# NeuralRevenant/RASSEngine

Measured on AMD Instinct MI355X. Metric: queries/sec, exact cosine top-10 over N x 1024-d fp32 corpus in HBM, higher is better.
Workload: dtype f32; 1 GPU; 1000000 x 1024-d flat cosine top-10, 1 x MI355X, precomputed embeddings (BASELINE configs[1]); rows_per_gpu=1000000, rows_global=1000000, dim=1024, k=10, query_batch=32, corpus_dtype=f32, layout=tile16, mode=flat

## Files before the change

include/rass_engine.h:

```cpp
#ifndef RASS_ENGINE_H
#define RASS_ENGINE_H

#include <stddef.h>
#include <stdint.h>

#ifdef __cplusplus
extern "C" {
#endif

#define RASS_ABI_VERSION 1

typedef enum rass_status {
    RASS_OK = 0,
    RASS_ERR_INVALID = -1,
    RASS_ERR_HIP = -2,
    RASS_ERR_OOM = -3,
    RASS_ERR_NOT_FOUND = -4,
    RASS_ERR_UNSUPPORTED = -5,
    RASS_ERR_IO = -6
} rass_status;

typedef enum rass_dtype {
    RASS_F32 = 0,
    RASS_BF16 = 1,
// ... 178 lines not shown
                                     const int32_t* d_q_filter, const int32_t* d_q_filter_mask,
                                     int64_t id_base, int32_t* d_out_groups, int64_t* d_out_counts, float* d_out_scores,
                                     int64_t* d_out_ids, int64_t* d_n_buckets, int64_t* d_total_hits, int32_t* d_status);

int rass_index_rows_gram(rass_index_t* idx, const int64_t* rows, int n_lists, int list_len, float* out);
int rass_index_rows_gram_device(rass_index_t* idx, const int64_t* d_rows, int n_lists, int list_len, float* d_out);

int rass_index_search_mmr(rass_index_t* idx, const float* queries, int nq, int k, int fetch_k,
                          const float* lambda, const int32_t* q_filter, const int32_t* q_filter_mask,
                          float* out_scores, int64_t* out_ids, int32_t* out_rank);
int rass_index_search_mmr_device(rass_index_t* idx, const float* d_queries, int nq, int k, int fetch_k,
                                 const float* d_lambda, const int32_t* d_q_filter, const int32_t* d_q_filter_mask,
                                 int64_t id_base, float* d_out_scores, int64_t* d_out_ids, int32_t* d_out_rank);

#define RASS_PREFILTER_OFF 0
#define RASS_PREFILTER_BF16 1
#define RASS_PREFILTER_INT8 2
#define RASS_PREFILTER_INT8_EXACT 3
int rass_index_set_prefilter(rass_index_t* idx, int enable);
int rass_index_get_prefilter(const rass_index_t* idx);
int rass_index_certify_stats(rass_index_t* idx, int64_t* queries, int64_t* certified, int64_t* fallbacks, float* R, float* V);
int rass_index_candidates_exact_device(rass_index_t* idx, const float* d_queries, int nq, int k, const int32_t* d_q_filter,
                                       float* d_cand_scores, int64_t* d_cand_rows, float* d_tau, int32_t* d_certified);
int rass_index_candidates_device(rass_index_t* idx, const float* d_queries, int nq, const int32_t* d_q_filter,
                                 float* d_cand_scores, int64_t* d_cand_rows);

int rass_index_save(rass_index_t* idx, const char* path);
int rass_index_load(rass_engine_t* eng, const char* name, const char* path,
                    rass_index_t** out);

int rass_index_fill_synthetic(rass_index_t* idx, int64_t n, uint64_t seed,
                              int64_t row_id_base);


size_t rass_scan_workspace_bytes(int nq, int k);

int rass_pack_rows_f32(const float* d_in, int64_t in_stride, float* d_packed,
                       int64_t row_stride, int64_t first_row, int64_t n, int dim,
                       int normalize, void* stream);
int rass_unpack_rows_f32(const float* d_packed, int64_t row_stride,
                         int64_t first_row, int64_t n, int dim, float* d_out,
                         int64_t out_stride, void* stream);
int rass_gather_rows_f32(const float* d_packed, int64_t row_stride, int64_t n_rows,
                         const int64_t* d_row_ids, int64_t n, int dim, float* d_out,
                         int64_t out_stride, void* stream);
int rass_compact_plan(const int32_t* d_tags, int64_t n_rows, int64_t* d_new_row,
// ... 191 lines not shown
```

rassengine_amd/_native.py:

```python
from __future__ import annotations

import ctypes
import os
from typing import Optional

_HERE = os.path.dirname(os.path.abspath(__file__))
LIB_PATH = os.environ.get("RASS_HIP_LIB") or os.path.join(_HERE, "lib", "librass_hip.so")

RASS_OK = 0
RASS_MAX_K = 32
RASS_MAX_K_MULTIPASS = 4096
RASS_TAG_PATIENT_MASK = 0x00FFFFFF
RASS_TAG_DOCTYPE_SHIFT = 24
RASS_TAG_DOCTYPE_MASK = 0x7F000000
RASS_MAX_QBATCH = 32
RASS_MAX_DEVICE_BATCH = 4096
RASS_MAX_MMR_FETCH = 128
RASS_F32 = 0
RASS_BF16 = 1
RASS_QFILTER_NONE = -1
RASS_MAX_ATTRS = 8
RASS_ATTR_MISSING = -(1 << 31)
RASS_MAX_ATTR_CLAUSES = 64
RASS_ATTR_ALL, RASS_ATTR_ANY = 0, 1
# ... 100 lines not shown
    "rass_index_attr_minmax": (ctypes.c_int, [ctypes.c_void_p, ctypes.c_int, ctypes.c_void_p, ctypes.c_void_p, ctypes.c_void_p]),
    "rass_index_search_grouped_keys": (ctypes.c_int, [ctypes.c_void_p, ctypes.c_void_p, ctypes.c_int, ctypes.c_int, ctypes.c_void_p, ctypes.c_int64, ctypes.c_int32, ctypes.c_void_p, ctypes.c_int, ctypes.c_int64, ctypes.c_void_p, ctypes.c_void_p, ctypes.c_void_p, ctypes.c_void_p, ctypes.c_void_p, ctypes.c_void_p]),
    "rass_index_search_grouped_keys_device": (ctypes.c_int, [ctypes.c_void_p, ctypes.c_void_p, ctypes.c_int, ctypes.c_int, ctypes.c_void_p, ctypes.c_int64, ctypes.c_int32, ctypes.c_void_p, ctypes.c_int, ctypes.c_int64, ctypes.c_void_p, ctypes.c_void_p, ctypes.c_int64, ctypes.c_void_p, ctypes.c_void_p, ctypes.c_void_p, ctypes.c_void_p, ctypes.c_void_p]),
    "rass_index_aggregate_keys": (ctypes.c_int, [ctypes.c_void_p, ctypes.c_void_p, ctypes.c_int, ctypes.c_void_p, ctypes.c_int, ctypes.c_void_p, ctypes.c_int64, ctypes.c_int32, ctypes.c_void_p, ctypes.c_int, ctypes.c_int64, ctypes.c_void_p, ctypes.c_void_p, ctypes.c_void_p, ctypes.c_void_p, ctypes.c_void_p, ctypes.c_void_p, ctypes.c_void_p, ctypes.c_void_p]),
    "rass_index_aggregate_keys_device": (ctypes.c_int, [ctypes.c_void_p, ctypes.c_void_p, ctypes.c_int, ctypes.c_void_p, ctypes.c_int, ctypes.c_void_p, ctypes.c_int64, ctypes.c_int32, ctypes.c_void_p, ctypes.c_int, ctypes.c_int64, ctypes.c_void_p, ctypes.c_void_p, ctypes.c_int64, ctypes.c_void_p, ctypes.c_void_p, ctypes.c_void_p, ctypes.c_void_p, ctypes.c_void_p, ctypes.c_void_p, ctypes.c_void_p]),
    "rass_index_rows_gram": (ctypes.c_int, [ctypes.c_void_p, ctypes.c_void_p, ctypes.c_int, ctypes.c_int, ctypes.c_void_p]),
    "rass_index_rows_gram_device": (ctypes.c_int, [ctypes.c_void_p, ctypes.c_void_p, ctypes.c_int, ctypes.c_int,
                                                   ctypes.c_void_p]),
    "rass_index_search_mmr": (ctypes.c_int, [ctypes.c_void_p, ctypes.c_void_p, ctypes.c_int, ctypes.c_int, ctypes.c_int,
                                             ctypes.c_void_p, ctypes.c_void_p, ctypes.c_void_p, ctypes.c_void_p, ctypes.c_void_p,
                                             ctypes.c_void_p]),
    "rass_index_search_mmr_device": (ctypes.c_int, [ctypes.c_void_p, ctypes.c_void_p, ctypes.c_int, ctypes.c_int, ctypes.c_int,
                                                    ctypes.c_void_p, ctypes.c_void_p, ctypes.c_void_p, ctypes.c_int64,
                                                    ctypes.c_void_p, ctypes.c_void_p, ctypes.c_void_p]),
    "rass_index_set_prefilter": (ctypes.c_int, [ctypes.c_void_p, ctypes.c_int]),
    "rass_index_get_prefilter": (ctypes.c_int, [ctypes.c_void_p]),
    "rass_index_candidates_device": (ctypes.c_int, [ctypes.c_void_p, ctypes.c_void_p, ctypes.c_int, ctypes.c_void_p,
                                                    ctypes.c_void_p, ctypes.c_void_p]),
    "rass_index_certify_stats": (ctypes.c_int, [ctypes.c_void_p, ctypes.c_void_p, ctypes.c_void_p, ctypes.c_void_p,
                                                ctypes.c_void_p, ctypes.c_void_p]),
    "rass_index_candidates_exact_device": (ctypes.c_int, [ctypes.c_void_p, ctypes.c_void_p, ctypes.c_int, ctypes.c_int,
                                                          ctypes.c_void_p, ctypes.c_void_p, ctypes.c_void_p, ctypes.c_void_p,
                                                          ctypes.c_void_p]),
    "rass_index_save": (ctypes.c_int, [ctypes.c_void_p, ctypes.c_char_p]),
    "rass_index_load": (ctypes.c_int, [ctypes.c_void_p, ctypes.c_char_p, ctypes.c_char_p, c_void_pp]),
    "rass_index_fill_synthetic": (ctypes.c_int, [ctypes.c_void_p, ctypes.c_int64, ctypes.c_uint64,
                                                 ctypes.c_int64]),
    "rass_scan_workspace_bytes": (ctypes.c_size_t, [ctypes.c_int, ctypes.c_int]),
    "rass_scan_topk_f32": (ctypes.c_int, [ctypes.c_void_p, ctypes.c_int64, ctypes.c_int, ctypes.c_int64,
                                          ctypes.c_void_p, ctypes.c_void_p, ctypes.c_int, ctypes.c_void_p,
                                          ctypes.c_int, ctypes.c_int64, ctypes.c_void_p, ctypes.c_void_p,
                                          ctypes.c_void_p, ctypes.c_size_t, ctypes.c_void_p]),
    "rass_pack_rows_f32": (ctypes.c_int, [ctypes.c_void_p, ctypes.c_int64, ctypes.c_void_p, ctypes.c_int64,
                                          ctypes.c_int64, ctypes.c_int64, ctypes.c_int, ctypes.c_int,
                                          ctypes.c_void_p]),
    "rass_unpack_rows_f32": (ctypes.c_int, [ctypes.c_void_p, ctypes.c_int64, ctypes.c_int64, ctypes.c_int64,
                                            ctypes.c_int, ctypes.c_void_p, ctypes.c_int64, ctypes.c_void_p]),
    "rass_gather_rows_f32": (ctypes.c_int, [ctypes.c_void_p, ctypes.c_int64, ctypes.c_int64, ctypes.c_void_p, ctypes.c_int64,
                                            ctypes.c_int, ctypes.c_void_p, ctypes.c_int64, ctypes.c_void_p]),
    "rass_compact_plan": (ctypes.c_int, [ctypes.c_void_p, ctypes.c_int64, ctypes.c_void_p, ctypes.c_void_p, ctypes.c_void_p,
                                         ctypes.c_void_p, ctypes.c_size_t, ctypes.c_void_p]),
    "rass_compact_plan_workspace_bytes": (ctypes.c_size_t, [ctypes.c_int64]),
    "rass_compact_rows_f32": (ctypes.c_int, [ctypes.c_void_p, ctypes.c_void_p, ctypes.c_int64, ctypes.c_void_p, ctypes.c_int64,
                                             ctypes.c_int64, ctypes.c_void_p]),
    "rass_topk_merge": (ctypes.c_int, [ctypes.c_void_p, ctypes.c_void_p, ctypes.c_int, ctypes.c_int, ctypes.c_int,
                                       ctypes.c_void_p, ctypes.c_void_p, ctypes.c_void_p]),
# ... 159 lines not shown
```

rassengine_amd/csrc/api_internal.h:

```cpp
#pragma once

#include <hip/hip_runtime.h>
#include <stdint.h>
#include <stdio.h>
#include <stdlib.h>
#include <string.h>
#include <unistd.h>

#include <algorithm>
#include <atomic>
#include <condition_variable>
#include <map>
#include <mutex>
#include <new>
#include <string>
#include <type_traits>
#include <vector>

#include "../../include/rass_engine.h"
#include "kernels.h"

namespace rass {
namespace host {

// ... 73 lines not shown
    }
};

struct ScratchView {
    float* q_padded;
    float* part_scores;
    int64_t* part_ids;
    unsigned short* q_bf16;
    float* cand_scores;
    int64_t* cand_ids;
    float* sample_best;
    size_t total;
};
ScratchView scratch_layout(unsigned char* base, int nq, int k);

struct BatchView {
    float* q_padded;
    float* part_scores;
    int64_t* part_ids;
    float* sample_best;
    unsigned char* q_small;
    float* cand_scores;
    int64_t* cand_rows;
    size_t total;
    size_t part_per_group;
    float* group_sample(int g) const { return sample_best + (int64_t)g * 32 * rass::kMaxSampleGroups; }
};
BatchView batch_layout(unsigned char* base, int groups, int grid, int k, int64_t stride, bool candidates = false);

struct CertView {
    float* q_padded;
    signed char* q8;
    rass::CertQInfo* qinfo;
    float* sample;
    float* list_s;
    int32_t* list_r;
    int32_t* list_n;
    float* list_floor;
    int64_t* cand_rows;
    float* rr_s;
    int64_t* rr_i;
    float* tau;
    int32_t *fail_idx, *fail_flag, *fail_n;
    float* fb_q;
    int32_t *fb_filter, *fb_mask;
    float* fb_s;
// ... 181 lines not shown
    uint32_t* d_list_mask = nullptr;
    bool any_tags = false;
    int64_t src_rows = 0;
    int64_t src_epoch = -1;
    std::vector<int32_t> pos_of;
    float* d_pair_scores = nullptr;
    int64_t* d_pair_ids = nullptr;
    unsigned char* d_batch = nullptr;
    size_t batch_bytes = 0;
};

namespace rass {
namespace host {

int set_device(const rass_engine* eng);
int index_reserve(rass_index* idx, int64_t need_rows);
void index_free_slabs(rass_index* idx);
int index_attr_ensure(rass_index* idx, int col);
int index_refresh_copies(rass_index* idx, int64_t first, int64_t n, hipStream_t st);

int scan_xcd_skew(int nq, int grid, int n_cus);
int64_t scan_sample_floor_min_share();
bool i8_sample_floor(int64_t rows, int grid);
bool scan_batch_one_sample();
bool scan_batch_pair();
bool ivf_batch_one_launch();

int scan_grid(int64_t tiles, int lists_kept_per_wg, int n_cus);

template <class F>
int timed_launch(rass_engine* eng, hipStream_t st, F&& launch, int extra_groups = 0) {
    const bool timed = eng && eng->ev_on && (size_t)(2 * eng->ev_used + 1) < eng->ev_pool.size();
    if (timed) HIP_TRY(hipEventRecord(eng->ev_pool[2 * eng->ev_used], st));
    const int rc = launch();
    if (rc != RASS_OK) return rc;
    if (timed) {
        HIP_TRY(hipEventRecord(eng->ev_pool[2 * eng->ev_used + 1], st));
        eng->ev_used += 1;
        eng->ev_extra += extra_groups;
    }
    return RASS_OK;
}

inline void as_sample(rass::ScanArgs& s) { s.xcd_skew = 0, s.sample_pass = true; }
inline void as_sample(rass::ScanBf16Args& s) { s.k = 1; }
inline void as_sample(rass::ScanI8Args& s) { s.k = 1; }
template <class Args>
// ... 142 lines not shown
```

rassengine_amd/csrc/api_scan.hip:

```cpp

#include "api_internal.h"

namespace rass {
namespace host {


int scan_xcd_skew(int nq, int grid, int n_cus) {
    struct Skew {
        int b16 = 4, b32 = 0;
        Skew() {
            if (const char* e = getenv("RASS_SCAN_XCD_SKEW")) {
                int a = 0, b = 0;
                const int n = sscanf(e, "%d,%d", &a, &b);
                if (n == 1) b = a;
                if (n >= 1 && a >= 0 && b >= 0 && a <= 4096 && b <= 4096) b16 = a, b32 = b;
            }
        }
    };
    if (grid != n_cus || grid % 8 != 0) return 0;
    static const Skew skew;
    return nq <= 16 ? skew.b16 : skew.b32;
}

int64_t scan_sample_floor_min_share() {
    const char* e = getenv("RASS_SCAN_SAMPLE_FLOOR");
    if (e && e[0] == '0') return 0;
    if (e && e[0] == 'f') return 2;
    return 32;
}

bool i8_sample_floor(int64_t rows, int grid) {
    const char* e = getenv("RASS_I8_SAMPLE_FLOOR");
    const bool force = e && e[0] == 'f';
    if (e && !force && atoi(e) == 0) return false;
    return grid <= rass::kMaxSampleGroups && rows >= (int64_t)(force ? 2 : 8) * 64 * grid;
}

bool scan_batch_one_sample() {
    const char* e = getenv("RASS_SCAN_BATCH_SAMPLE");
    return !(e && e[0] == 'g');
}

bool scan_batch_pair() {
    static const bool on = [] {
        const char* e = getenv("RASS_SCAN_BATCH_PAIR");
        return !(e && e[0] == '0');
    }();
    return on;
}

bool ivf_batch_one_launch() {
    const char* e = getenv("RASS_IVF_BATCH_FINE");
    return !(e && e[0] == 'g');
}


int scan_grid(int64_t tiles, int lists_kept_per_wg, int n_cus) {
    int grid = (int)std::min<int64_t>(std::max<int64_t>(tiles, 1), std::min(n_cus, kMaxGrid));
    if ((int64_t)grid * lists_kept_per_wg > rass::kMergeMaxCandidates) grid = rass::kMergeMaxCandidates / lists_kept_per_wg;
    return grid;
}

ScratchView scratch_layout(unsigned char* base, int nq, int k) {
// ... 1 lines not shown
    ScratchView L;
    L.q_padded = c.take<float>((size_t)RASS_MAX_QBATCH * kMaxStride * sizeof(float));
    L.part_scores = c.take<float>((size_t)kMaxGrid * nq * k * sizeof(float));
    L.part_ids = c.take<int64_t>((size_t)kMaxGrid * nq * k * sizeof(int64_t));
    L.q_bf16 = c.take<unsigned short>((size_t)RASS_MAX_QBATCH * kMaxStride * 2);
    L.cand_scores = c.take<float>((size_t)RASS_MAX_QBATCH * RASS_MAX_K * sizeof(float));
    L.cand_ids = c.take<int64_t>((size_t)RASS_MAX_QBATCH * RASS_MAX_K * sizeof(int64_t));
    L.sample_best = c.take<float>((size_t)rass::kMaxSampleGroups * 32 * sizeof(float));
    L.total = c.off;
    return L;
}

BatchView batch_layout(unsigned char* base, int groups, int grid, int k, int64_t stride, bool candidates) {
    Carver c{base};
    BatchView L;
    L.part_per_group = (size_t)grid * 32 * k;
    L.q_padded = c.take<float>((size_t)groups * 32 * stride * sizeof(float));
    L.part_scores = c.take<float>((size_t)groups * L.part_per_group * sizeof(float));
    L.part_ids = c.take<int64_t>((size_t)groups * L.part_per_group * sizeof(int64_t));
    L.sample_best = c.take<float>((size_t)groups * 32 * rass::kMaxSampleGroups * sizeof(float));
    L.q_small = candidates ? c.take<unsigned char>((size_t)groups * 32 * kMaxStride * 2) : nullptr;
    L.cand_scores = candidates ? c.take<float>((size_t)groups * 32 * k * sizeof(float)) : nullptr;
    L.cand_rows = candidates ? c.take<int64_t>((size_t)groups * 32 * k * sizeof(int64_t)) : nullptr;
    L.total = c.off;
    return L;
}

CertView cert_layout(unsigned char* base, int grid, int64_t stride, int64_t stride_i8, int dim) {
    Carver c{base};
    CertView L;
    const size_t Q = rass::kCertQ, slots = (size_t)grid * Q * rass::kCertWgCap;
    L.q_padded = c.take<float>(4 * Q * stride * sizeof(float));
    L.q8 = c.take<signed char>(2 * Q * stride_i8);
    L.qinfo = c.take<rass::CertQInfo>(Q * sizeof(rass::CertQInfo));
    L.sample = c.take<float>((size_t)rass::kMaxSampleGroups * Q * sizeof(float));
    L.list_s = c.take<float>(slots * sizeof(float));
    L.list_r = c.take<int32_t>(slots * sizeof(int32_t));
    L.list_n = c.take<int32_t>((size_t)grid * Q * sizeof(int32_t));
    L.list_floor = c.take<float>((size_t)grid * Q * sizeof(float));
    L.cand_rows = c.take<int64_t>(Q * rass::kCertC * sizeof(int64_t));
    L.rr_s = c.take<float>(Q * rass::kCertC * sizeof(float));
    L.rr_i = c.take<int64_t>(Q * rass::kCertC * sizeof(int64_t));
    L.tau = c.take<float>(Q * sizeof(float));
    L.fail_idx = c.take<int32_t>(Q * sizeof(int32_t));
    L.fail_flag = c.take<int32_t>(Q * sizeof(int32_t));
    L.fail_n = c.take<int32_t>(sizeof(int32_t));
// ... 394 lines not shown
```

rassengine_amd/csrc/api_search.hip:

```cpp

#include "api_internal.h"

namespace rass {
namespace host {

HostSlot* slot_acquire(rass_engine* eng) {
    std::unique_lock<std::mutex> lk(eng->slot_mu);
    for (;;) {
        for (HostSlot& sl : eng->slots)
            if (!sl.busy) {
                sl.busy = true;
                return &sl;
            }
        eng->slot_cv.wait(lk);
    }
}

void slot_release(rass_engine* eng, HostSlot* sl) {
    {
        std::lock_guard<std::mutex> lk(eng->slot_mu);
        sl->busy = false;
    }
    eng->slot_cv.notify_one();
}
// ... 38 lines not shown
    const IndexView iv = index_view(idx, r.q_filter != nullptr, r.id_base, r.after_score != nullptr);
    r.use(iv);
    if (idx->dtype == RASS_BF16) return bf16_scan_launch(idx, r);
    if (!exact && idx->prefilter == 3 && iv.rows > 0 && !r.after_score && one_pass) return cert_launch(idx, r);
    if (!exact && idx->prefilter && idx->prefilter != 3 && iv.rows > 0 && r.k <= kPrefilterMaxK && !r.after_score)
        return prefilter_launch(idx, r);
    ScanRequest s = scan_request(eng);
    s.corpus = iv.corpus, s.n_rows = iv.rows, s.stride = idx->stride, s.row_tag = iv.row_tag;
    s.queries = r.queries, s.q_dim = idx->dim, s.q_stride = idx->dim, s.nq = r.nq, s.q_filter = r.q_filter;
    s.k = r.k, s.id_base = iv.id_base, s.id_map = iv.id_map, s.out_scores = r.out_scores, s.out_ids = r.out_ids;
    s.timing = eng;
    s.ext.d_q_mask = r.q_filter_mask, s.ext.d_after_s = r.after_score, s.ext.d_after_i = r.after_row;
    return scan_launch(s);
}

FlatRequest batch_group(const rass_index* idx, const FlatRequest& r, int g, int64_t gs, int64_t gi) {
    FlatRequest q = r;
    q.nq = std::min(RASS_MAX_QBATCH, r.nq - g * RASS_MAX_QBATCH);
    q.queries = r.queries + (int64_t)g * RASS_MAX_QBATCH * idx->dim;
    q.q_filter = r.q_filter ? r.q_filter + g * RASS_MAX_QBATCH : nullptr;
    q.out_scores = r.out_scores + g * gs;
    q.out_ids = r.out_ids + g * gi;
    return q;
}

int scan_launch_batch(rass_index* idx, const FlatRequest& r, int64_t gs, int64_t gi) {
    rass_engine* eng = idx->eng;
    hipStream_t st = eng->stream;
    const int nq = r.nq, k = r.k;
    const IndexView iv = index_view(idx, r.q_filter != nullptr, r.id_base);
    const int64_t rows = iv.rows;
    const int64_t stride = idx->stride;
    if (int rc = check_k(k)) return rc;
    if (rows < 0 || rows > kMaxScanRows) return fail(RASS_ERR_INVALID, "n_rows out of range for one scan");
    if (!rass::scan_supported_stride(stride) || stride > kMaxStride)
        return fail(RASS_ERR_UNSUPPORTED, kStrideMsg);
    const int groups = (nq + RASS_MAX_QBATCH - 1) / RASS_MAX_QBATCH;
    if (stride > kNarrowStride) {
        for (int g = 0; g < groups; ++g) {
            const int rc = search_device_group(idx, batch_group(idx, r, g, gs, gi));
            if (rc != RASS_OK) return rc;
        }
        return RASS_OK;
    }
    const int grid = scan_grid((rows + 31) / 32, k, eng->n_cus);
    int rc = grow_block(&eng->d_batch, &eng->batch_bytes, batch_layout(nullptr, groups, grid, k, stride).total, st);
    if (rc != RASS_OK) return rc;
    const BatchView L = batch_layout(eng->d_batch, groups, grid, k, stride);

    HIP_TRY(rass::launch_normalize_rows_f32(r.queries, idx->dim, L.q_padded, stride, nq, idx->dim, st, (int64_t)groups * 32));

    auto group_args = [&](int g) {
        rass::ScanArgs a;
        a.corpus = iv.corpus;
        a.row_tag = iv.row_tag;
        a.q_padded = L.q_padded + (int64_t)g * 32 * stride;
        a.q_filter = r.q_filter ? r.q_filter + g * 32 : nullptr;
        a.part_scores = L.part_scores + (int64_t)g * L.part_per_group;
        a.part_ids = L.part_ids + (int64_t)g * L.part_per_group;
        a.row_stride = stride;
        a.id_base = iv.id_base;
        a.n_rows = (int)rows;
        a.nq = std::min(RASS_MAX_QBATCH, nq - g * 32);
        a.k = k;
        a.xcd_skew = scan_xcd_skew(a.nq, grid, eng->n_cus);
        return a;
    };
    const int64_t sample_rows = (int64_t)64 * grid;
    const int64_t min_share = scan_sample_floor_min_share();
    const bool sample = min_share > 0 && grid <= rass::kMaxSampleGroups && rows >= min_share * sample_rows;
    const bool one_sample = sample && groups >= 2 && nq % 32 == 0 && scan_batch_one_sample() && grid >= 32;
    const int sample_wgs = one_sample ? 32 : grid;
    if (one_sample) {
        rass::ScanArgs s = group_args(0);
        s.n_rows = (int)sample_rows;
        s.xcd_skew = 0;
        s.sample_pass = true;
        s.nq = 32;
        s.part_scores = L.sample_best;
        s.part_ids = nullptr;
        s.wgs_per_group = sample_wgs;
        s.q_group_stride = 32 * stride;
        s.part_group_stride = (int64_t)32 * rass::kMaxSampleGroups;
        s.nq_total = nq;
        HIP_TRY(rass::launch_scan_topk_f32(s, groups * sample_wgs, st));
    } else if (sample)
        for (int g = 0; g < groups; ++g) {
            rass::ScanArgs a = group_args(g);
            if (a.nq <= 16) continue;
            rc = sample_prelaunch(a, grid, L.group_sample(g), rass::launch_scan_topk_f32, st);
            if (rc != RASS_OK) return rc;
        }
    const bool pairs = scan_batch_pair() && rass::scan_pair_supported_stride(stride);
    for (int g = 0; g < groups; ++g) {
        rass::ScanArgs a = group_args(g);
        if (sample && a.nq > 16) {
            a.sample_best = L.group_sample(g);
            a.sample_groups = sample_wgs;
        }
        const bool pair = pairs && a.nq == RASS_MAX_QBATCH && (g + 2) * RASS_MAX_QBATCH <= nq;
        if (pair) {
            a.nq = 2 * RASS_MAX_QBATCH;
            a.q_group_stride = 32 * stride;
            a.part_group_stride = (int64_t)L.part_per_group;
            a.xcd_skew = scan_xcd_skew(a.nq, grid, eng->n_cus);
            rc = timed_launch(eng, st, [&] { return HIP_RC(rass::launch_scan_topk_f32_pair(a, grid, st)); }, 1);
            ++g;
        } else
            rc = timed_launch(eng, st, [&] { return HIP_RC(rass::launch_scan_topk_f32(a, grid, st)); });
        if (rc != RASS_OK) return rc;
    }
    const rass::MergeGroups mg = dense_groups(nq, (int64_t)L.part_per_group, gs, gi);
    HIP_TRY(rass::launch_merge_topk(L.part_scores, L.part_ids, grid, nq, k, r.out_scores, r.out_ids, st, iv.id_map, 0, 0, &mg));
    return RASS_OK;
}

int prefilter_launch_batch(rass_index* idx, const FlatRequest& r, int64_t gs, int64_t gi) {
    rass_engine* eng = idx->eng;
    hipStream_t st = eng->stream;
    const int nq = r.nq;
    const IndexView iv = index_view(idx, r.q_filter != nullptr, r.id_base);
    const int64_t rows = iv.rows;
    const int64_t stride = idx->stride;
    const int kc = RASS_MAX_K;
    const int groups = (nq + RASS_MAX_QBATCH - 1) / RASS_MAX_QBATCH;
    const int grid = scan_grid((rows + 63) / 64, kc, eng->n_cus);
    int rc = grow_block(&eng->d_batch, &eng->batch_bytes, batch_layout(nullptr, groups, grid, kc, stride, true).total, st);
    if (rc != RASS_OK) return rc;
    const BatchView L = batch_layout(eng->d_batch, groups, grid, kc, stride, true);
    const int nq_pad = groups * 32;
    HIP_TRY(rass::launch_normalize_rows_f32(r.queries, idx->dim, L.q_padded, stride, nq, idx->dim, st, nq_pad));
    const bool i8 = idx->prefilter == 2;
    const int64_t qs_stride = i8 ? idx->stride_i8 : stride * 2;
    if (i8) HIP_TRY(rass::launch_queries_to_i8(L.q_padded, L.q_small, nq_pad, stride, idx->stride_i8, st));
    else HIP_TRY(rass::launch_queries_to_bf16(L.q_padded, L.q_small, (int64_t)nq_pad * stride, st));
    const bool floor_on = i8_sample_floor(rows, grid);
    const bool one_sample = i8 && floor_on && groups >= 2 && nq % 32 == 0;
    if (one_sample) {
        rass::ScanI8Args all = i8_args(idx, rows, iv.row_tag, kc);
// ... 204 lines not shown
    if (certified) *certified = (int64_t)c[1];
    if (fallbacks) *fallbacks = (int64_t)c[2];
    if (R) *R = f[0];
    if (V) *V = f[1];
    return RASS_OK;
}

int rass_index_candidates_exact_device(rass_index_t* idx, const float* d_queries, int nq, int k, const int32_t* d_q_filter,
                                       float* d_cand_scores, int64_t* d_cand_rows, float* d_tau, int32_t* d_certified) {
    if (!idx || !d_queries || !d_cand_scores || !d_cand_rows || !d_tau || !d_certified) return fail(RASS_ERR_INVALID, "NULL argument");
    if (int rc = check_nq(nq)) return rc;
    if (int rc = check_k(k)) return rc;
    rass_engine* eng = idx->eng;
    std::lock_guard<std::mutex> lk(eng->mu);
    int rc = set_device(eng);
    if (rc != RASS_OK) return rc;
    if (idx->prefilter != 3 || idx->dtype != RASS_F32) return fail(RASS_ERR_UNSUPPORTED, "the index is not in prefilter mode 3");
    if (idx->rows.load(std::memory_order_acquire) <= 0) return fail(RASS_ERR_INVALID, "the index is empty");
    FlatRequest r;
    r.queries = d_queries, r.nq = nq, r.k = k, r.q_filter = d_q_filter;
    r.row_tag = index_view(idx, d_q_filter != nullptr).row_tag;
    r.cand_scores = d_cand_scores, r.cand_rows = d_cand_rows, r.tau = d_tau, r.certified = d_certified;
    return cert_launch(idx, r);
}

int rass_index_search_ex(rass_index_t* idx, const float* queries, int nq, int k, const int32_t* q_filter,
                         const int32_t* q_filter_mask, float* out_scores, int64_t* out_ids) {
    if (!idx || !out_scores || !out_ids) return fail(RASS_ERR_INVALID, "NULL argument");
    if (nq < 0 || (nq > 0 && !queries)) return fail(RASS_ERR_INVALID, "bad queries / nq");
    if (k < 1 || k > RASS_MAX_K_MULTIPASS) return fail(RASS_ERR_INVALID, "k must be in [1, RASS_MAX_K_MULTIPASS]");
    if (q_filter_mask && !q_filter) return fail(RASS_ERR_INVALID, "q_filter_mask without q_filter");
    return one_layout([&] { return idx->layout_epoch.load(std::memory_order_acquire); },
                      [&] { return search_ex_once(idx, queries, nq, k, q_filter, q_filter_mask, out_scores, out_ids); });
}

static int search_multi_once(rass_engine* eng, rass_index_t* const* idxs, const float* queries, int nq, int k,
                             const int32_t* q_filter, const int32_t* q_filter_mask, float* out_scores, int64_t* out_ids) {
    int rc = set_device(eng);
    if (rc != RASS_OK) return rc;
    const int dim = eng->dim;
    SlotGuard guard(eng);
    HostSlot* sl = guard.sl;
    const size_t item_bytes = 4 + 4 + 4 + 8 + 8;
    if (!sl->h_items) HIP_TRY(hipHostMalloc(&sl->h_items, (size_t)kMultiMaxItems * item_bytes, hipHostMallocDefault));
    int32_t* h_tile = static_cast<int32_t*>(sl->h_items);
    int32_t* h_rows = h_tile + kMultiMaxItems;
// ... 118 lines not shown
```

rassengine_amd/csrc/kernels.h:

```cpp
#pragma once

#include <hip/hip_runtime.h>
#include <stddef.h>
#include <stdint.h>

namespace rass {

constexpr int kMaxSampleGroups = 256;

struct ScanArgs {
    const float* corpus;
    const int32_t* row_tag;
    const float* q_padded;
    const int32_t* q_filter;
    const int32_t* q_filter_mask = nullptr;
    const float* q_after_score = nullptr;
    const int64_t* q_after_id = nullptr;
    float* part_scores;
    int64_t* part_ids;
    int64_t row_stride;
    int64_t id_base;
    int n_rows;
    int nq;
    int k;
// ... 115 lines not shown
    int64_t* part_ids;
    int64_t row_stride;
    int n_rows;
    int nq;
    int k;
    int64_t id_base = 0;
    const int32_t* q_filter_mask = nullptr;
    const float* q_after_score = nullptr;
    const int64_t* q_after_id = nullptr;
    const int32_t* work_tile = nullptr;
    const int32_t* work_rows = nullptr;
    const uint32_t* work_mask = nullptr;
    const int32_t* n_work = nullptr;
    const float* sample_best = nullptr;
    int sample_groups = 0;
};
hipError_t launch_scan_bf16_topk(const ScanBf16Args& a, int grid, hipStream_t stream);
hipError_t launch_convert_tile16_bf16(const float* src, void* dst, int64_t stride, int64_t block0, int64_t block1,
                                      hipStream_t stream, int64_t src_block0 = -1, int64_t row_lo = 0,
                                      int64_t row_hi = -1);
hipError_t launch_unpack_rows_tile16b(const void* slab, int64_t stride, int64_t first_row, int64_t n, int dim,
                                      float* out, int64_t out_stride, hipStream_t stream);
hipError_t launch_queries_to_bf16(const float* src, void* dst, int64_t n, hipStream_t stream);
hipError_t launch_rerank_f32(const float* slab, int64_t stride, const float* q_padded, const int64_t* cand_rows, int nq,
                             int n_cand, int k, int64_t id_base, float* out_scores, int64_t* out_ids,
                             hipStream_t stream, int64_t out_scores_group_stride = 0, int64_t out_ids_group_stride = 0,
                             const int64_t* id_map = nullptr);

struct ScanI8Args {
    const signed char* corpus;
    const float* row_scale;
    const int32_t* row_tag;
    const signed char* q_i8;
    const int32_t* q_filter;
    float* part_scores;
    int64_t* part_ids;
    int64_t row_stride;
    int n_rows;
    int nq;
    int k;
    const float* sample_best = nullptr;
    int sample_groups = 0;
    const int32_t* q_filter_mask = nullptr;
    int wgs_per_group = 0;
    int64_t q_group_stride = 0, part_group_stride = 0;
    const int32_t* work_tile = nullptr;
// ... 155 lines not shown
```

rassengine_amd/csrc/scan_bf16.hip:

```cpp

#include <hip/hip_runtime.h>
#include <hip/hip_bf16.h>
#include <stdint.h>

#include "kernels.h"
#include "scan_core.h"

namespace rass {

typedef short bf16x8 __attribute__((ext_vector_type(8)));
typedef unsigned short u16;

constexpr int kBWaves = 8;
constexpr int kBThreads = kBWaves * 64;
constexpr int kBTileRows = 64;
constexpr int kBPitch = 68;

__device__ __forceinline__ u16 f2bf_s(float f) {
    __hip_bfloat16 h = __float2bfloat16(f);
    return *reinterpret_cast<u16*>(&h);
}

struct BDesc {
    __amdgpu_buffer_rsrc_t rows;
    __amdgpu_buffer_rsrc_t tags;
};

struct BWork {
    int tile, rows;
// ... 325 lines not shown

hipError_t launch_queries_to_bf16(const float* src, void* dst, int64_t n, hipStream_t stream) {
    if (n <= 0) return hipSuccess;
    int64_t blocks = (n + 255) / 256;
    if (blocks > 1024) blocks = 1024;
    hipLaunchKernelGGL(queries_to_bf16_kernel, dim3((unsigned)blocks), dim3(256), 0, stream, src, static_cast<u16*>(dst), n);
    return hipGetLastError();
}

template <int CH, int HALVES>
__device__ __forceinline__ void rerank_f32_body(const float* __restrict__ slab, int64_t stride, const float* __restrict__ q_padded,
                                                const int64_t* __restrict__ cand_rows, int n_cand, int k, int64_t id_base,
                                                float* __restrict__ out_scores, int64_t* __restrict__ out_ids, int64_t gs, int64_t gi,
                                                const int64_t* __restrict__ id_map) {
    __shared__ float part[32][9];
    __shared__ float sc[32];
    __shared__ int64_t rw[32];
    const int q = blockIdx.x;
    float* const os = out_scores + (gs > 0 ? (int64_t)(q >> 5) * gs + (int64_t)(q & 31) * k : (int64_t)q * k);
    int64_t* const oi = out_ids + (gi > 0 ? (int64_t)(q >> 5) * gi + (int64_t)(q & 31) * k : (int64_t)q * k);
    const int c = threadIdx.x >> 3, w = threadIdx.x & 7;
    const int64_t row = c < n_cand ? cand_rows[(int64_t)q * n_cand + c] : -1;
    float acc = 0.f;
    if (row >= 0) {
#pragma unroll
        for (int half = 0; half < HALVES; ++half) {
            const float* xb = slab + (row >> 4) * 16 * stride + (int64_t)(w * HALVES * CH + half * CH) * 256 + (int)(row & 15) * 4;
            const float* qv = q_padded + (int64_t)q * stride + (w * HALVES * CH + half * CH) * 16;
            f32x4 xv[CH][4];
#pragma unroll
            for (int j = 0; j < CH; ++j)
#pragma unroll
                for (int g = 0; g < 4; ++g) xv[j][g] = *reinterpret_cast<const f32x4*>(xb + j * 256 + g * 64);
#pragma unroll
            for (int j = 0; j < CH; ++j) {
                f32x4 qq[4];
#pragma unroll
                for (int g = 0; g < 4; ++g) qq[g] = *reinterpret_cast<const f32x4*>(qv + j * 16 + 4 * g);
#pragma unroll
                for (int i = 0; i < 4; ++i)
#pragma unroll
                    for (int g = 0; g < 4; ++g) acc = fmaf(xv[j][g][i], qq[g][i], acc);
            }
        }
    }
    part[c][w] = acc;
    __syncthreads();
    if (threadIdx.x < 32) {
        const int cc = threadIdx.x;
        float s = part[cc][0];
#pragma unroll
        for (int ww = 1; ww < 8; ++ww) s += part[cc][ww];
        const int64_t r = cc < n_cand ? cand_rows[(int64_t)q * n_cand + cc] : -1;
        sc[cc] = r >= 0 ? s : -INFINITY;
        rw[cc] = (r >= 0 && id_map != nullptr) ? id_map[r] : r;
    }
    __syncthreads();
    if (threadIdx.x < 32) {
        const int cc = threadIdx.x;
        const float s = sc[cc];
        const int64_t r = rw[cc];
        int rank = 0;
        for (int o = 0; o < 32; ++o) {
            const float so = sc[o];
            const int64_t ro = rw[o];
            const bool o_valid = ro >= 0, me_valid = r >= 0;
            const bool better = o_valid && (!me_valid || so > s || (so == s && ro < r));
            rank += (o != cc && better) ? 1 : 0;
// ... 65 lines not shown
```

rassengine_amd/engine.py:

```python
from __future__ import annotations

import ctypes
import threading
from typing import Dict, Optional, Tuple

import numpy as np

from . import _native as N


def _np_ptr(a: Optional[np.ndarray]):
    return None if a is None else a.ctypes.data_as(ctypes.c_void_p)


def pack_allow(mask: np.ndarray) -> np.ndarray:
    m = np.asarray(mask, dtype=bool)
    if m.ndim not in (1, 2):
        raise ValueError(f"expected a boolean mask [n] or [nb, n], got shape {m.shape}")
    n = m.shape[-1]
    words = (n + 31) // 32
    padded = np.zeros(m.shape[:-1] + (words * 32,), dtype=bool)
    padded[..., :n] = m
    packed = np.packbits(padded, axis=-1, bitorder="little")
    return np.ascontiguousarray(packed).view("<u4").reshape(m.shape[:-1] + (words,)).astype(np.uint32, copy=False)
# ... 243 lines not shown
                                                 ctypes.byref(R), ctypes.byref(V)))
        return {"queries": q.value, "certified": c.value, "fallbacks": f.value, "R": R.value, "V": V.value}

    def candidates_exact_device(self, d_queries, k: int, q_filter=None):
        import torch
        nq = int(d_queries.shape[0])
        assert d_queries.is_cuda and d_queries.dtype == torch.float32 and d_queries.is_contiguous() and d_queries.shape[1] == self.dim
        dev = d_queries.device
        s = torch.empty((nq, 128), dtype=torch.float32, device=dev)
        r = torch.empty((nq, 128), dtype=torch.int64, device=dev)
        tau = torch.empty((nq,), dtype=torch.float32, device=dev)
        cert = torch.empty((nq,), dtype=torch.int32, device=dev)
        f = None
        if q_filter is not None:
            f = torch.as_tensor(np.ascontiguousarray(q_filter, dtype=np.int32)).to(dev)
        torch.cuda.current_stream().synchronize()
        N.check("rass_index_candidates_exact_device",
                self._L.rass_index_candidates_exact_device(self._h, ctypes.c_void_p(d_queries.data_ptr()), nq, int(k),
                                                           ctypes.c_void_p(f.data_ptr()) if f is not None else None,
                                                           ctypes.c_void_p(s.data_ptr()), ctypes.c_void_p(r.data_ptr()),
                                                           ctypes.c_void_p(tau.data_ptr()), ctypes.c_void_p(cert.data_ptr())))
        self.engine.synchronize()
        return s, r, tau, cert

    def candidates_device(self, d_queries, q_filter=None):
        import torch
        nq = int(d_queries.shape[0])
        assert d_queries.is_cuda and d_queries.dtype == torch.float32 and d_queries.is_contiguous() and d_queries.shape[1] == self.dim
        s = torch.empty((nq, 32), dtype=torch.float32, device=d_queries.device)
        r = torch.empty((nq, 32), dtype=torch.int64, device=d_queries.device)
        f = None
        if q_filter is not None:
            f = torch.as_tensor(np.ascontiguousarray(q_filter, dtype=np.int32)).to(d_queries.device)
        torch.cuda.current_stream().synchronize()
        N.check("rass_index_candidates_device",
                self._L.rass_index_candidates_device(self._h, ctypes.c_void_p(d_queries.data_ptr()), nq,
                                                     ctypes.c_void_p(f.data_ptr()) if f is not None else None,
                                                     ctypes.c_void_p(s.data_ptr()), ctypes.c_void_p(r.data_ptr())))
        self.engine.synchronize()
        return s, r

    def save(self, path: str) -> None:
        N.check("rass_index_save", self._L.rass_index_save(self._h, path.encode()))

    def _queries(self, queries) -> np.ndarray:
        q = np.ascontiguousarray(queries, dtype=np.float32)
# ... 669 lines not shown
```

Measured before the change: 59530 queries/s.

## Compute batch sample floor with bf16 MFMA representatives plus exact fp32 rescore

Adds a new default sample-floor stage for batched fp32 flat scans. A bf16 MFMA kernel scores a 64-row sample per workgroup against all queries and keeps the best representative row per query and block. A second kernel rescores those representatives exactly in fp32 to set the per-group sample floor. This replaces the previous fp32 one-sample scan launch, aiming to cut the cost of the pruning-threshold pass, at the price of extra launches and workspace. Also adds a debug API that exposes the floor, and factors the exact scoring routine into a shared header.

Result: faster. 60230 queries/s, median of 6 (+1.2%).

```diff
diff --git a/include/rass_engine.h b/include/rass_engine.h
--- a/include/rass_engine.h
+++ b/include/rass_engine.h
@@ -224,6 +224,8 @@
 int rass_index_certify_stats(rass_index_t* idx, int64_t* queries, int64_t* certified, int64_t* fallbacks, float* R, float* V);
 int rass_index_candidates_exact_device(rass_index_t* idx, const float* d_queries, int nq, int k, const int32_t* d_q_filter,
                                        float* d_cand_scores, int64_t* d_cand_rows, float* d_tau, int32_t* d_certified);
+int rass_index_sample_floor_device(rass_index_t* idx, const float* d_queries, int nq, int k, const int32_t* d_q_filter,
+                                   int32_t* d_out_rows, float* d_out_scores);
 int rass_index_candidates_device(rass_index_t* idx, const float* d_queries, int nq, const int32_t* d_q_filter,
                                  float* d_cand_scores, int64_t* d_cand_rows);
 
diff --git a/rassengine_amd/_native.py b/rassengine_amd/_native.py
--- a/rassengine_amd/_native.py
+++ b/rassengine_amd/_native.py
@@ -146,6 +146,8 @@
     "rass_index_candidates_exact_device": (ctypes.c_int, [ctypes.c_void_p, ctypes.c_void_p, ctypes.c_int, ctypes.c_int,
                                                           ctypes.c_void_p, ctypes.c_void_p, ctypes.c_void_p, ctypes.c_void_p,
                                                           ctypes.c_void_p]),
+    "rass_index_sample_floor_device": (ctypes.c_int, [ctypes.c_void_p, ctypes.c_void_p, ctypes.c_int, ctypes.c_int,
+                                                      ctypes.c_void_p, ctypes.c_void_p, ctypes.c_void_p]),
     "rass_index_save": (ctypes.c_int, [ctypes.c_void_p, ctypes.c_char_p]),
     "rass_index_load": (ctypes.c_int, [ctypes.c_void_p, ctypes.c_char_p, ctypes.c_char_p, c_void_pp]),
     "rass_index_fill_synthetic": (ctypes.c_int, [ctypes.c_void_p, ctypes.c_int64, ctypes.c_uint64,
diff --git a/rassengine_amd/csrc/api_internal.h b/rassengine_amd/csrc/api_internal.h
--- a/rassengine_amd/csrc/api_internal.h
+++ b/rassengine_amd/csrc/api_internal.h
@@ -119,6 +119,9 @@
     unsigned char* q_small;
     float* cand_scores;
     int64_t* cand_rows;
+    unsigned char* rep_qfrag;
+    unsigned char* rep_part;
+    int* rep_row;
     size_t total;
     size_t part_per_group;
     float* group_sample(int g) const { return sample_best + (int64_t)g * 32 * rass::kMaxSampleGroups; }
@@ -346,7 +349,8 @@
 int scan_xcd_skew(int nq, int grid, int n_cus);
 int64_t scan_sample_floor_min_share();
 bool i8_sample_floor(int64_t rows, int grid);
-bool scan_batch_one_sample();
+enum { kBatchSampleGroups = 0, kBatchSampleF32 = 1, kBatchSampleRep = 2 };
+int scan_batch_sample_mode();
 bool scan_batch_pair();
 bool ivf_batch_one_launch();
 
diff --git a/rassengine_amd/csrc/api_scan.hip b/rassengine_amd/csrc/api_scan.hip
--- a/rassengine_amd/csrc/api_scan.hip
+++ b/rassengine_amd/csrc/api_scan.hip
@@ -36,9 +36,11 @@
     return grid <= rass::kMaxSampleGroups && rows >= (int64_t)(force ? 2 : 8) * 64 * grid;
 }
 
-bool scan_batch_one_sample() {
+int scan_batch_sample_mode() {
     const char* e = getenv("RASS_SCAN_BATCH_SAMPLE");
-    return !(e && e[0] == 'g');
+    if (e && e[0] == 'g') return kBatchSampleGroups;
+    if (e && e[0] == 'f') return kBatchSampleF32;
+    return kBatchSampleRep;
 }
 
 bool scan_batch_pair() {
@@ -86,6 +88,9 @@
     L.q_small = candidates ? c.take<unsigned char>((size_t)groups * 32 * kMaxStride * 2) : nullptr;
     L.cand_scores = candidates ? c.take<float>((size_t)groups * 32 * k * sizeof(float)) : nullptr;
     L.cand_rows = candidates ? c.take<int64_t>((size_t)groups * 32 * k * sizeof(int64_t)) : nullptr;
+    L.rep_qfrag = candidates ? nullptr : c.take<unsigned char>((size_t)groups * 32 * stride * 2);
+    L.rep_part = candidates ? nullptr : c.take<unsigned char>((size_t)groups * 32 * rass::kMaxSampleGroups * 8);
+    L.rep_row = candidates ? nullptr : c.take<int>((size_t)groups * 32 * 32 * sizeof(int));
     L.total = c.off;
     return L;
 }
diff --git a/rassengine_amd/csrc/api_search.hip b/rassengine_amd/csrc/api_search.hip
--- a/rassengine_amd/csrc/api_search.hip
+++ b/rassengine_amd/csrc/api_search.hip
@@ -84,6 +84,22 @@
     q.out_scores = r.out_scores + g * gs;
     q.out_ids = r.out_ids + g * gi;
     return q;
+}
+
+struct BatchSamplePlan {
+    int grid;
+    bool sample, one_sample, rep;
+};
+BatchSamplePlan batch_sample_plan(const rass_engine* eng, int64_t rows, int64_t stride, int nq, int k) {
+    BatchSamplePlan p;
+    p.grid = scan_grid((rows + 31) / 32, k, eng->n_cus);
+    const int groups = (nq + RASS_MAX_QBATCH - 1) / RASS_MAX_QBATCH;
+    const int64_t min_share = scan_sample_floor_min_share();
+    const int mode = scan_batch_sample_mode();
+    p.sample = min_share > 0 && p.grid <= rass::kMaxSampleGroups && rows >= min_share * 64 * p.grid;
+    p.one_sample = p.sample && groups >= 2 && nq % 32 == 0 && mode != kBatchSampleGroups && p.grid >= 32;
+    p.rep = p.one_sample && mode == kBatchSampleRep && rass::sample_rep_supported(stride, p.grid);
+    return p;
 }
 
 int scan_launch_batch(rass_index* idx, const FlatRequest& r, int64_t gs, int64_t gi) {
@@ -105,7 +121,8 @@
         }
         return RASS_OK;
     }
-    const int grid = scan_grid((rows + 31) / 32, k, eng->n_cus);
+    const BatchSamplePlan plan = batch_sample_plan(eng, rows, stride, nq, k);
+    const int grid = plan.grid;
     int rc = grow_block(&eng->d_batch, &eng->batch_bytes, batch_layout(nullptr, groups, grid, k, stride).total, st);
     if (rc != RASS_OK) return rc;
     const BatchView L = batch_layout(eng->d_batch, groups, grid, k, stride);
@@ -129,11 +146,12 @@
         return a;
     };
     const int64_t sample_rows = (int64_t)64 * grid;
-    const int64_t min_share = scan_sample_floor_min_share();
-    const bool sample = min_share > 0 && grid <= rass::kMaxSampleGroups && rows >= min_share * sample_rows;
-    const bool one_sample = sample && groups >= 2 && nq % 32 == 0 && scan_batch_one_sample() && grid >= 32;
+    const bool sample = plan.sample, one_sample = plan.one_sample;
     const int sample_wgs = one_sample ? 32 : grid;
-    if (one_sample) {
+    if (plan.rep) {
+        HIP_TRY(rass::launch_sample_rep(iv.corpus, iv.row_tag, stride, grid, L.q_padded, r.q_filter, nq, L.rep_qfrag, L.rep_part,
+                                        L.rep_row, L.sample_best, st));
+    } else if (one_sample) {
         rass::ScanArgs s = group_args(0);
         s.n_rows = (int)sample_rows;
         s.xcd_skew = 0;
@@ -177,6 +195,30 @@
     return RASS_OK;
 }
 
+int sample_floor_hook(rass_index* idx, const float* d_queries, int nq, int k, const int32_t* d_q_filter, int32_t* d_rows,
+                      float* d_scores) {
+    rass_engine* eng = idx->eng;
+    hipStream_t st = eng->stream;
+    const IndexView iv = index_view(idx, d_q_filter != nullptr, 0);
+    const int64_t stride = idx->stride;
+    if (idx->dtype != RASS_F32 || idx->prefilter || nq <= RASS_MAX_QBATCH || iv.rows <= 0 || iv.rows > kMaxScanRows ||
+        stride > kNarrowStride || !rass::scan_supported_stride(stride))
+        return fail(RASS_ERR_UNSUPPORTED, "not a fused fp32 batch");
+    const BatchSamplePlan plan = batch_sample_plan(eng, iv.rows, stride, nq, k);
+    if (!plan.rep) return fail(RASS_ERR_UNSUPPORTED, "this batch does not take the representatives' sample stage");
+    const int groups = nq / RASS_MAX_QBATCH;
+    int rc = grow_block(&eng->d_batch, &eng->batch_bytes, batch_layout(nullptr, groups, plan.grid, k, stride).total, st);
+    if (rc != RASS_OK) return rc;
+    const BatchView L = batch_layout(eng->d_batch, groups, plan.grid, k, stride);
+    HIP_TRY(rass::launch_normalize_rows_f32(d_queries, idx->dim, L.q_padded, stride, nq, idx->dim, st, nq));
+    HIP_TRY(rass::launch_sample_rep(iv.corpus, iv.row_tag, stride, plan.grid, L.q_padded, d_q_filter, nq, L.rep_qfrag, L.rep_part,
+                                    L.rep_row, L.sample_best, st));
+    HIP_TRY(hipMemcpyAsync(d_rows, L.rep_row, (size_t)nq * 32 * sizeof(int32_t), hipMemcpyDeviceToDevice, st));
+    HIP_TRY(hipMemcpy2DAsync(d_scores, 32 * sizeof(float), L.sample_best, rass::kMaxSampleGroups * sizeof(float), 32 * sizeof(float),
+                             (size_t)nq, hipMemcpyDeviceToDevice, st));
+    return RASS_OK;
+}
+
 int prefilter_launch_batch(rass_index* idx, const FlatRequest& r, int64_t gs, int64_t gi) {
     rass_engine* eng = idx->eng;
     hipStream_t st = eng->stream;
@@ -427,6 +469,18 @@
     r.row_tag = index_view(idx, d_q_filter != nullptr).row_tag;
     r.cand_scores = d_cand_scores, r.cand_rows = d_cand_rows, r.tau = d_tau, r.certified = d_certified;
     return cert_launch(idx, r);
+}
+
+int rass_index_sample_floor_device(rass_index_t* idx, const float* d_queries, int nq, int k, const int32_t* d_q_filter,
+                                   int32_t* d_out_rows, float* d_out_scores) {
+    if (!idx || !d_queries || !d_out_rows || !d_out_scores) return fail(RASS_ERR_INVALID, "NULL argument");
+    if (nq < 1 || nq > RASS_MAX_DEVICE_BATCH) return fail(RASS_ERR_INVALID, "nq must be in [1, RASS_MAX_DEVICE_BATCH]");
+    if (int rc = check_k(k)) return rc;
+    rass_engine* eng = idx->eng;
+    std::lock_guard<std::mutex> lk(eng->mu);
+    int rc = set_device(eng);
+    if (rc != RASS_OK) return rc;
+    return sample_floor_hook(idx, d_queries, nq, k, d_q_filter, d_out_rows, d_out_scores);
 }
 
 int rass_index_search_ex(rass_index_t* idx, const float* queries, int nq, int k, const int32_t* q_filter,
diff --git a/rassengine_amd/csrc/exact_score.h b/rassengine_amd/csrc/exact_score.h
--- /dev/null
+++ b/rassengine_amd/csrc/exact_score.h
@@ -0,0 +1,37 @@
+#pragma once
+
+#include <hip/hip_runtime.h>
+#include <stdint.h>
+
+#include "scan_core.h"
+
+namespace rass {
+
+template <int CH, int HALVES>
+__device__ __forceinline__ float flat_score_slice(const float* __restrict__ slab, int64_t stride, const float* __restrict__ q_padded,
+                                                  int q, int64_t row, int w) {
+    float acc = 0.f;
+#pragma unroll
+    for (int half = 0; half < HALVES; ++half) {
+        const float* xb = slab + (row >> 4) * 16 * stride + (int64_t)(w * HALVES * CH + half * CH) * 256 + (int)(row & 15) * 4;
+        const float* qv = q_padded + (int64_t)q * stride + (w * HALVES * CH + half * CH) * 16;
+        f32x4 xv[CH][4];
+#pragma unroll
+        for (int j = 0; j < CH; ++j)
+#pragma unroll
+            for (int g = 0; g < 4; ++g) xv[j][g] = *reinterpret_cast<const f32x4*>(xb + j * 256 + g * 64);
+#pragma unroll
+        for (int j = 0; j < CH; ++j) {
+            f32x4 qq[4];
+#pragma unroll
+            for (int g = 0; g < 4; ++g) qq[g] = *reinterpret_cast<const f32x4*>(qv + j * 16 + 4 * g);
+#pragma unroll
+            for (int i = 0; i < 4; ++i)
+#pragma unroll
+                for (int g = 0; g < 4; ++g) acc = fmaf(xv[j][g][i], qq[g][i], acc);
+        }
+    }
+    return acc;
+}
+
+}
diff --git a/rassengine_amd/csrc/kernels.h b/rassengine_amd/csrc/kernels.h
--- a/rassengine_amd/csrc/kernels.h
+++ b/rassengine_amd/csrc/kernels.h
@@ -161,6 +161,10 @@
 hipError_t launch_unpack_rows_tile16b(const void* slab, int64_t stride, int64_t first_row, int64_t n, int dim,
                                       float* out, int64_t out_stride, hipStream_t stream);
 hipError_t launch_queries_to_bf16(const float* src, void* dst, int64_t n, hipStream_t stream);
+bool sample_rep_supported(int64_t stride, int grid);
+hipError_t launch_sample_rep(const float* slab, const int32_t* row_tag, int64_t stride, int grid, const float* q_padded,
+                             const int32_t* q_filter, int nq, void* q_frag, void* rep_part, int* rep_row, float* sample_best,
+                             hipStream_t stream);
 hipError_t launch_rerank_f32(const float* slab, int64_t stride, const float* q_padded, const int64_t* cand_rows, int nq,
                              int n_cand, int k, int64_t id_base, float* out_scores, int64_t* out_ids,
                              hipStream_t stream, int64_t out_scores_group_stride = 0, int64_t out_ids_group_stride = 0,
diff --git a/rassengine_amd/csrc/sample_rep.hip b/rassengine_amd/csrc/sample_rep.hip
--- /dev/null
+++ b/rassengine_amd/csrc/sample_rep.hip
@@ -0,0 +1,222 @@
+
+#include <hip/hip_runtime.h>
+#include <limits.h>
+#include <stdint.h>
+
+#include "kernels.h"
+#include "scan_core.h"
+#include "exact_score.h"
+
+namespace rass {
+
+typedef __bf16 bf16x8 __attribute__((ext_vector_type(8)));
+typedef __bf16 bf16x4 __attribute__((ext_vector_type(4)));
+
+constexpr int kRepThreads = 512;
+constexpr int kRepRows = 64;
+
+__device__ __forceinline__ bf16x8 pack_bf16(const f32x4 a, const f32x4 b) {
+    const bf16x4 lo = __builtin_convertvector(a, bf16x4), hi = __builtin_convertvector(b, bf16x4);
+    return __builtin_shufflevector(lo, hi, 0, 1, 2, 3, 4, 5, 6, 7);
+}
+
+__device__ __forceinline__ void take_better(float& s, int& r, float os, int orow) {
+    const bool take = (os > s) | ((os == s) & (orow < r));
+    s = take ? os : s;
+    r = take ? orow : r;
+}
+
+__global__ __launch_bounds__(256) void sample_queries_frag_kernel(const float* __restrict__ q_padded, int64_t stride,
+                                                                  bf16x8* __restrict__ q_frag, int n_frag) {
+    const int i = blockIdx.x * 256 + threadIdx.x;
+    if (i >= n_frag) return;
+    const int ks_per_tile = (int)(stride >> 5);
+    const int lane = i & 63, ks = (i >> 6) % ks_per_tile, tile = (i >> 6) / ks_per_tile;
+    const float* src = q_padded + (int64_t)(tile * 16 + (lane & 15)) * stride + 32 * ks + 4 * (lane >> 4);
+    q_frag[i] = pack_bf16(*reinterpret_cast<const f32x4*>(src), *reinterpret_cast<const f32x4*>(src + 16));
+}
+
+template <int CH>
+__global__ __launch_bounds__(kRepThreads, 2) void sample_rep_bf16_kernel(const float* __restrict__ slab,
+                                                                         const int32_t* __restrict__ row_tag,
+                                                                         const bf16x8* __restrict__ q_frag,
+                                                                         const int32_t* __restrict__ q_filter, int n_tiles,
+                                                                         int2* __restrict__ rep_part) {
+    constexpr int KS = 4 * CH;
+    constexpr int64_t stride = 128 * CH;
+    __shared__ bf16x8 rows[KS * 4 * 64];
+    const int lane = threadIdx.x & 63;
+    const int wid = __builtin_amdgcn_readfirstlane(threadIdx.x >> 6);
+    const int g = lane >> 4;
+    const int row0 = blockIdx.x * kRepRows;
+
+    {
+        const float* base = slab + (int64_t)row0 * stride + lane * 4;
+#pragma unroll
+        for (int half = 0; half < 2; ++half) {
+            f32x4 v[CH][2];
+#pragma unroll
+            for (int u = 0; u < CH; ++u) {
+                const int item = wid + 8 * (half * CH + u), rb = item / KS, ks = item % KS;
+                const float* c = base + (int64_t)rb * 16 * stride + ks * 512;
+                v[u][0] = *reinterpret_cast<const f32x4*>(c);
+                v[u][1] = *reinterpret_cast<const f32x4*>(c + 256);
+            }
+#pragma unroll
+            for (int u = 0; u < CH; ++u) {
+                const int item = wid + 8 * (half * CH + u), rb = item / KS, ks = item % KS;
+                rows[(ks * 4 + rb) * 64 + lane] = pack_bf16(v[u][0], v[u][1]);
+            }
+        }
+    }
+    const __amdgpu_buffer_rsrc_t trs = make_rsrc(reinterpret_cast<uint64_t>(row_tag ? row_tag + row0 : nullptr), row_tag ? kRepRows * 4u : 0u);
+    const __amdgpu_buffer_rsrc_t frs = make_rsrc(reinterpret_cast<uint64_t>(q_filter), q_filter ? (unsigned)n_tiles * 64u : 0u);
+    int tag[4][4];
+#pragma unroll
+    for (int rb = 0; rb < 4; ++rb)
+#pragma unroll
+        for (int r = 0; r < 4; ++r) tag[rb][r] = (int)__builtin_amdgcn_raw_buffer_load_b32(trs, (16 * rb + 4 * g + r) * 4, 0, 0);
+    __syncthreads();
+    if (wid >= n_tiles) return;
+
+    bf16x8 qf[KS];
+    int t = wid;
+    {
+        const bf16x8* qp = q_frag + (int64_t)t * KS * 64 + lane;
+#pragma unroll
+        for (int ks = 0; ks < KS; ++ks) {
+            __builtin_amdgcn_sched_barrier(0);
+            qf[ks] = qp[ks * 64];
+        }
+        __builtin_amdgcn_sched_barrier(0);
+    }
+
+    do {
+        asm volatile("" ::: "memory");
+        const int q = t * 16 + (lane & 15);
+        const int qraw = (int)__builtin_amdgcn_raw_buffer_load_b32(frs, q * 4, 0, 0);
+        __builtin_amdgcn_sched_barrier(0);
+        const bf16x8* qn = q_frag + (int64_t)min(t + 8, n_tiles - 1) * KS * 64 + lane;
+        f32x4 acc[4];
+#pragma unroll
+        for (int rb = 0; rb < 4; ++rb) acc[rb] = f32x4{0.f, 0.f, 0.f, 0.f};
+        bf16x8 a[3][4];
+#pragma unroll
+        for (int pre = 0; pre < 2; ++pre)
+#pragma unroll
+            for (int rb = 0; rb < 4; ++rb) a[pre][rb] = rows[(pre * 4 + rb) * 64 + lane];
+#pragma unroll
+        for (int ks = 0; ks < KS; ++ks) {
+            if (ks + 2 < KS) {
+#pragma unroll
+                for (int rb = 0; rb < 4; ++rb) a[(ks + 2) % 3][rb] = rows[((ks + 2) * 4 + rb) * 64 + lane];
+            }
+#pragma unroll
+            for (int rb = 0; rb < 4; ++rb)
+                acc[rb] = __builtin_amdgcn_mfma_f32_16x16x32_bf16(a[ks % 3][rb], qf[ks], acc[rb], 0, 0, 0);
+            qf[ks] = qn[ks * 64];
+            __builtin_amdgcn_sched_barrier(0);
+        }
+        const int qfil = q_filter ? qraw : -1;
+        float bs = -INFINITY;
+        int br = INT_MAX;
+#pragma unroll
+        for (int rb = 0; rb < 4; ++rb)
+#pragma unroll
+            for (int r = 0; r < 4; ++r) {
+                const int tg = tag[rb][r];
+                const bool ok = (tg != -1) & ((qfil < 0) | (qfil == tg));
+                const float s = acc[rb][r];
+                const bool take = ok & (s > bs);
+                bs = take ? s : bs;
+                br = take ? row0 + 16 * rb + 4 * g + r : br;
+            }
+        take_better(bs, br, __int_as_float(xor_lane<16>(__float_as_int(bs), lane)), xor_lane<16>(br, lane));
+        take_better(bs, br, __int_as_float(xor_lane<32>(__float_as_int(bs), lane)), xor_lane<32>(br, lane));
+        if (lane < 16) rep_part[(int64_t)q * gridDim.x + blockIdx.x] = make_int2(__float_as_int(bs), br);
+        t += 8;
+    } while (t < n_tiles);
+}
+
+template <int CH>
+__global__ __launch_bounds__(256) __attribute__((amdgpu_waves_per_eu(1, 2))) void sample_rescore_f32_kernel(const float* __restrict__ slab,
+                                                                 const float* __restrict__ q_padded,
+                                                                 const int2* __restrict__ rep_part, int grid, int n_groups,
+                                                                 int* __restrict__ rep_row, float* __restrict__ sample_best) {
+    constexpr int64_t stride = 128 * CH;
+    __shared__ float part[32][9];
+    __shared__ int rw[32];
+    const int x = blockIdx.x & 7, j = blockIdx.x >> 3;
+    const int c = threadIdx.x >> 3, w = threadIdx.x & 7;
+    const int subs = grid >> 5;
+    const int lane = lane_id();
+    if (j >= n_groups) return;
+    auto pick = [&](int b, int grp) {
+        float bs = -INFINITY;
+        int br = INT_MAX;
+        if (w < subs) {
+            const int2 v = rep_part[(int64_t)(grp * 32 + c) * grid + b * subs + w];
+            bs = __int_as_float(v.x), br = v.y;
+        }
+        take_better(bs, br, __int_as_float(xor_lane<1>(__float_as_int(bs), lane)), xor_lane<1>(br, lane));
+        take_better(bs, br, __int_as_float(xor_lane<2>(__float_as_int(bs), lane)), xor_lane<2>(br, lane));
+        take_better(bs, br, __int_as_float(xor_lane<4>(__float_as_int(bs), lane)), xor_lane<4>(br, lane));
+        return br == INT_MAX ? -1 : br;
+    };
+    int b = x, grp = j;
+    int row = pick(b, grp);
+    for (;;) {
+        int nb = b, ng = grp + 32;
+        if (ng >= n_groups) nb = b + 8, ng = j;
+        const bool more = nb < 32;
+        const int row_next = more ? pick(nb, ng) : -1;
+        float acc = 0.f;
+        if (row >= 0) acc = flat_score_slice<CH, 1>(slab, stride, q_padded, grp * 32 + c, row, w);
+        part[c][w] = acc;
+        if (w == 0) rw[c] = row;
+        __syncthreads();
+        if (threadIdx.x < 32) {
+            const int cc = threadIdx.x, qq = grp * 32 + cc;
+            float s = part[cc][0];
+#pragma unroll
+            for (int ww = 1; ww < 8; ++ww) s += part[cc][ww];
+            const int r = rw[cc];
+            const bool ok = r >= 0 && fabsf(s) < INFINITY;
+            sample_best[(int64_t)qq * kMaxSampleGroups + b] = ok ? s : -INFINITY;
+            rep_row[qq * 32 + b] = r;
+        }
+        if (!more) break;
+        __syncthreads();
+        b = nb, grp = ng, row = row_next;
+    }
+}
+
+bool sample_rep_supported(int64_t stride, int grid) {
+    return stride >= 128 && stride <= 1024 && stride % 128 == 0 && grid >= 32 && grid % 32 == 0 && grid <= kMaxSampleGroups;
+}
+
+hipError_t launch_sample_rep(const float* slab, const int32_t* row_tag, int64_t stride, int grid, const float* q_padded,
+                             const int32_t* q_filter, int nq, void* q_frag, void* rep_part, int* rep_row, float* sample_best,
+                             hipStream_t stream) {
+    if (!sample_rep_supported(stride, grid) || nq < 32 || nq % 32 != 0) return hipErrorInvalidValue;
+    bf16x8* const qf = static_cast<bf16x8*>(q_frag);
+    int2* const part = static_cast<int2*>(rep_part);
+    const int n_frag = (int)((int64_t)nq * stride / 8);
+    hipLaunchKernelGGL(sample_queries_frag_kernel, dim3((n_frag + 255) / 256), dim3(256), 0, stream, q_padded, stride, qf, n_frag);
+#define RASS_REP_CASE(C)                                                                                                      \
+    case C:                                                                                                                   \
+        hipLaunchKernelGGL(sample_rep_bf16_kernel<C>, dim3(grid), dim3(kRepThreads), 0, stream, slab, row_tag, qf, q_filter,  \
+                           nq / 16, part);                                                                                    \
+        hipLaunchKernelGGL(sample_rescore_f32_kernel<C>, dim3(256), dim3(256), 0, stream, slab, q_padded, part, grid, nq / 32, \
+                           rep_row, sample_best);                                                                             \
+        break;
+    switch ((int)(stride >> 7)) {
+        RASS_REP_CASE(1) RASS_REP_CASE(2) RASS_REP_CASE(3) RASS_REP_CASE(4)
+        RASS_REP_CASE(5) RASS_REP_CASE(6) RASS_REP_CASE(7) RASS_REP_CASE(8)
+        default: return hipErrorInvalidValue;
+    }
+#undef RASS_REP_CASE
+    return hipGetLastError();
+}
+
+}
diff --git a/rassengine_amd/csrc/scan_bf16.hip b/rassengine_amd/csrc/scan_bf16.hip
--- a/rassengine_amd/csrc/scan_bf16.hip
+++ b/rassengine_amd/csrc/scan_bf16.hip
@@ -5,6 +5,7 @@
 
 #include "kernels.h"
 #include "scan_core.h"
+#include "exact_score.h"
 
 namespace rass {
 
@@ -376,28 +377,7 @@
     const int c = threadIdx.x >> 3, w = threadIdx.x & 7;
     const int64_t row = c < n_cand ? cand_rows[(int64_t)q * n_cand + c] : -1;
     float acc = 0.f;
-    if (row >= 0) {
-#pragma unroll
-        for (int half = 0; half < HALVES; ++half) {
-            const float* xb = slab + (row >> 4) * 16 * stride + (int64_t)(w * HALVES * CH + half * CH) * 256 + (int)(row & 15) * 4;
-            const float* qv = q_padded + (int64_t)q * stride + (w * HALVES * CH + half * CH) * 16;
-            f32x4 xv[CH][4];
-#pragma unroll
-            for (int j = 0; j < CH; ++j)
-#pragma unroll
-                for (int g = 0; g < 4; ++g) xv[j][g] = *reinterpret_cast<const f32x4*>(xb + j * 256 + g * 64);
-#pragma unroll
-            for (int j = 0; j < CH; ++j) {
-                f32x4 qq[4];
-#pragma unroll
-                for (int g = 0; g < 4; ++g) qq[g] = *reinterpret_cast<const f32x4*>(qv + j * 16 + 4 * g);
-#pragma unroll
-                for (int i = 0; i < 4; ++i)
-#pragma unroll
-                    for (int g = 0; g < 4; ++g) acc = fmaf(xv[j][g][i], qq[g][i], acc);
-            }
-        }
-    }
+    if (row >= 0) acc = flat_score_slice<CH, HALVES>(slab, stride, q_padded, q, row, w);
     part[c][w] = acc;
     __syncthreads();
     if (threadIdx.x < 32) {
diff --git a/rassengine_amd/engine.py b/rassengine_amd/engine.py
--- a/rassengine_amd/engine.py
+++ b/rassengine_amd/engine.py
@@ -289,6 +289,24 @@
                                                            ctypes.c_void_p(tau.data_ptr()), ctypes.c_void_p(cert.data_ptr())))
         self.engine.synchronize()
         return s, r, tau, cert
+
+    def sample_floor_device(self, d_queries, k: int, q_filter=None):
+        import torch
+        nq = int(d_queries.shape[0])
+        assert d_queries.is_cuda and d_queries.dtype == torch.float32 and d_queries.is_contiguous() and d_queries.shape[1] == self.dim
+        dev = d_queries.device
+        rows = torch.empty((nq, 32), dtype=torch.int32, device=dev)
+        scores = torch.empty((nq, 32), dtype=torch.float32, device=dev)
+        f = None
+        if q_filter is not None:
+            f = torch.as_tensor(np.ascontiguousarray(q_filter, dtype=np.int32)).to(dev)
+        torch.cuda.current_stream().synchronize()
+        N.check("rass_index_sample_floor_device",
+                self._L.rass_index_sample_floor_device(self._h, ctypes.c_void_p(d_queries.data_ptr()), nq, int(k),
+                                                       ctypes.c_void_p(f.data_ptr()) if f is not None else None,
+                                                       ctypes.c_void_p(rows.data_ptr()), ctypes.c_void_p(scores.data_ptr())))
+        self.engine.synchronize()
+        return rows, scores
 
     def candidates_device(self, d_queries, q_filter=None):
         import torch
```
